# kerry-he/fsae-mpc

Measured on AMD Instinct MI355X. Metric: QP solves/sec (batched LTV-MPC, N=40 nx=5 nu=2 fp64), higher is better.
Workload: dtype f64

## Files before the change

fsae-mpc_amd/csrc/qp_solver.hip:

```cpp
#include <hip/hip_runtime.h>
#include <math.h>
#include <stdint.h>
#include <stdlib.h>
#include <stdio.h>
#include "qp_solver.h"

typedef double v4d __attribute__((ext_vector_type(4)));
typedef double v2d __attribute__((ext_vector_type(2)));

#define DEVINL __device__ __forceinline__
#ifndef QP_SOLVE_REFINE_STEPS
#define QP_SOLVE_REFINE_STEPS 1
#endif
#ifndef QP_FULL_BARRIERS
#define WAVE_SYNC() do { __builtin_amdgcn_fence(__ATOMIC_SEQ_CST, "wavefront"); __builtin_amdgcn_wave_barrier(); } while (0)
#else
#define WAVE_SYNC() __syncthreads()
#endif

namespace {

DEVINL double rl(double v, int src) {
  int lo = __builtin_amdgcn_readlane(__double2loint(v), src);
  int hi = __builtin_amdgcn_readlane(__double2hiint(v), src);
// ... 327 lines not shown
        int rank, size; group(k, on, rank, size);
        int base = on ? cnt[w][k] : 0;
        if (on) order[base + rank] = i0 + 64 * r + lane;
        if (on && rank == 0) cnt[w][k] = base + size;
      }
    }
}

#endif

struct Ctx {
  int n, m, T, Kq, J, JB, JT, np, ld, lane, c, q, nc, nb, ntr;
  const int* perm; const int* tcs; const int* aoff; const int* tend;
  const double* Aw; const double* Hw; const double* Ab; const double* Hb;
  double* rows;
  double* ring;
  double* cof;
  int rowlen;
  double* Ms;
  double* vec;
};
enum VecArr { V_X = 0, V_G, V_HX, V_R1, V_R2, V_P1, V_P2, V_P3, V_DX, V_E, V_NARR };

DEVINL double* rowp(const Ctx& k, int arr) { return k.rows + (size_t)arr * k.rowlen; }
DEVINL double* vecp(const Ctx& k, int arr) { return k.vec + arr * k.np; }

DEVINL bool row_valid(const Ctx& k, int js) {
  if (js < k.J) { const int s = 16 * js + k.c; return s < k.Kq && 4 * s + k.q < k.m; }
  return (js - k.J) * 64 + k.lane < k.n;
}

template <int T> DEVINL void hx_tiles(const Ctx& k, const double* X, double* HX) {
  double hx[T], hn[T][4], hc[T][4];
#pragma unroll
  for (int t = 0; t < T; ++t) hx[t] = 0.0;
#pragma unroll
  for (int Jt = 0; Jt < T; ++Jt)
#pragma unroll
    for (int p = 0; p < 4; ++p) hn[Jt][p] = k.Hw[((size_t)Jt * 4 + p) * 64 + k.lane];
#pragma unroll 1
  for (int I = 0; I < T; ++I) {
#pragma unroll
    for (int Jt = 0; Jt < T; ++Jt)
#pragma unroll
      for (int p = 0; p < 4; ++p) hc[Jt][p] = hn[Jt][p];
    if (I + 1 < T) {
#pragma unroll
      for (int Jt = 0; Jt < T; ++Jt)
#pragma unroll
        for (int p = 0; p < 4; ++p) hn[Jt][p] = k.Hw[((size_t)((I + 1) * T + Jt) * 4 + p) * 64 + k.lane];
    }
    double xk[4];
#pragma unroll
    for (int p = 0; p < 4; ++p) xk[p] = X[16 * I + k.q + 4 * p];
#pragma unroll
    for (int Jt = 0; Jt < T; ++Jt)
#pragma unroll
      for (int p = 0; p < 4; ++p) hx[Jt] = fma(hc[Jt][p], xk[p], hx[Jt]);
  }
#pragma unroll
  for (int t = 0; t < T; ++t) {
    double v = q_sum(hx[t]);
    if (k.q == 0) HX[16 * t + k.c] = v;
  }
}
template <int T> DEVINL void acc_init(const Ctx& k, v4d* acc) {
#pragma unroll
  for (int I = 0; I < T; ++I)
#pragma unroll
    for (int Jt = I; Jt < T; ++Jt) {
      const double* hp = k.Hw + ((size_t)(I * T + Jt) * 4) * 64 + k.lane;
      v4d h;
#pragma unroll
      for (int p = 0; p < 4; ++p) h[p] = hp[p * 64];
      acc[Tri<T>::idx(I, Jt)] = h;
    }
}

template <int T> DEVINL void hx_from_acc(const Ctx& k, const v4d* acc, const double* XV, double* HX) {
  double xr[T][4], xc[T], sc[T], sr[T][4];
#pragma unroll
  for (int I = 0; I < T; ++I) {
    xc[I] = XV[16 * I + k.c]; sc[I] = 0.0;
#pragma unroll
    for (int p = 0; p < 4; ++p) { xr[I][p] = XV[16 * I + k.q + 4 * p]; sr[I][p] = 0.0; }
  }
#pragma unroll
  for (int I = 0; I < T; ++I)
#pragma unroll
    for (int J = I; J < T; ++J) {
      const v4d& h = acc[Tri<T>::idx(I, J)];
#pragma unroll
      for (int p = 0; p < 4; ++p) {
        sc[J] = fma(h[p], xr[I][p], sc[J]);
        if (J > I) sr[I][p] = fma(h[p], xc[J], sr[I][p]);
      }
    }
  WAVE_SYNC();
#pragma unroll
  for (int J = 0; J < T; ++J) { const double v = q_sum(sc[J]); if (k.q == 0) HX[16 * J + k.c] = v; }
  WAVE_SYNC();
#pragma unroll
  for (int I = 0; I < T - 1; ++I)
#pragma unroll
    for (int p = 0; p < 4; ++p) { const double v = grp16_sum(sr[I][p]); if (k.c == 0) HX[16 * I + k.q + 4 * p] += v; }
}

template <int C> struct IC { static constexpr int value = C; };

#ifdef QP_DRAIN_STREAM
template <int T> struct StreamCfg {
  static constexpr int R = 3 * T;
};
template <int T> struct Stream {
  static constexpr int R = StreamCfg<T>::R;
  const char* gnext;
  int half;
  DEVINL void issue(const Ctx& k, int slot) {
    __builtin_amdgcn_global_load_lds((const __attribute__((address_space(1))) void*)(gnext + k.lane * 16),
                                     (__attribute__((address_space(3))) void*)(k.ring + slot * 128), 16, 0, 0);
    gnext += 1024;
  }
  DEVINL void start(const Ctx& k, int c0) {
    gnext = reinterpret_cast<const char*>(k.Aw); half = 0;
#pragma unroll
    for (int t = 0; t < T; ++t) if (t < c0) issue(k, t);
  }
  template <int C> DEVINL void next_pair(const Ctx& k, v2d* b, int cn) {
    asm volatile("s_waitcnt vmcnt(0)" ::: "memory");
    const int other = (half ^ 1) * T;
#pragma unroll
    for (int t = 0; t < T; ++t) if (t < cn) issue(k, other + t);
    asm volatile("" ::: "memory");
#pragma unroll
    for (int t = 0; t < C; ++t) b[t] = *reinterpret_cast<const v2d*>(k.ring + (half * T + t) * 128 + k.lane * 2);
    half ^= 1;
  }
  DEVINL void drain() { asm volatile("s_waitcnt vmcnt(0)" ::: "memory"); }
};
#else
template <int T> struct StreamCfg {
  static constexpr int D = 2 * T;
  static constexpr int R = D + T;
};
template <int T> struct Stream {
  static constexpr int D = StreamCfg<T>::D, R = StreamCfg<T>::R;
  const char* gnext; int slot_i, slot_e;
  DEVINL void issue(const Ctx& k) {
    __builtin_amdgcn_global_load_lds((const __attribute__((address_space(1))) void*)(gnext + k.lane * 16),
                                     (__attribute__((address_space(3))) void*)(k.ring + slot_i * 128), 16, 0, 0);
    gnext += 1024;
    slot_i = slot_i + 1 == R ? 0 : slot_i + 1;
  }
  DEVINL void start(const Ctx& k, int) {
    gnext = reinterpret_cast<const char*>(k.Aw); slot_i = 0; slot_e = 0;
#pragma unroll
    for (int j = 0; j < D; ++j) issue(k);
  }
  template <int C> DEVINL void next_pair(const Ctx& k, v2d* b, int) {
#pragma unroll
    for (int t = 0; t < C; ++t) issue(k);
    asm volatile("s_waitcnt vmcnt(%0)" :: "n"(D) : "memory");
#pragma unroll
    for (int t = 0; t < C; ++t) {
      int sl = slot_e + t; if (sl >= R) sl -= R;
      b[t] = *reinterpret_cast<const v2d*>(k.ring + sl * 128 + k.lane * 2);
    }
    slot_e += C; if (slot_e >= R) slot_e -= R;
  }
  DEVINL void drain() { asm volatile("s_waitcnt vmcnt(0)" ::: "memory"); }
};
#endif

template <int NA> struct CoefStage {
  double reg[NA > 0 ? NA : 1];
  DEVINL void load(const Ctx& k, const double* const* arr, int js) {
    const int jc = js < k.J ? js : k.J - 1;
#pragma unroll
    for (int a = 0; a < NA; ++a) reg[a] = arr[a][jc * 64 + k.lane];
  }
  DEVINL void commit(const Ctx& k) {
#pragma unroll
    for (int a = 0; a < NA; ++a) k.cof[a * 64 + k.lane] = reg[a];
  }
  DEVINL void read_pair(const Ctx& k, int s, v2d* out) const {
#pragma unroll
    for (int a = 0; a < NA; ++a) out[a] = *reinterpret_cast<const v2d*>(k.cof + a * 64 + k.q * 16 + (s & 15));
  }
};

template <int T, int NB> DEVINL void pass_syrk(const Ctx& k, v4d* acc, double* P1, double* P2, double* P3, double* MB) {
  constexpr int NBB = NB > 0 ? NB : 1;
  constexpr int NA = 4 + NB;
  const int JS = k.J * 64;
  const double* arr[NA];
  arr[0] = rowp(k, R_D); arr[1] = rowp(k, R_W1); arr[2] = rowp(k, R_W2); arr[3] = rowp(k, R_W3);
#pragma unroll
  for (int e = 0; e < NB; ++e) arr[4 + e] = k.Ab + (size_t)e * JS;
  double p1[T], p2[T], p3[T];
  double pb[NBB][T], sbb[NBB][NBB], pwb[3][NBB];
#pragma unroll
  for (int t = 0; t < T; ++t) { p1[t] = 0; p2[t] = 0; p3[t] = 0; }
#pragma unroll
  for (int e = 0; e < NBB; ++e) {
#pragma unroll
    for (int t = 0; t < T; ++t) pb[e][t] = 0;
#pragma unroll
    for (int f = 0; f < NBB; ++f) sbb[e][f] = 0;
    pwb[0][e] = pwb[1][e] = pwb[2][e] = 0;
  }
  Stream<T> st;
  CoefStage<NA> cs;
  int tr = 0;
  if (k.ntr > 0) { st.start(k, k.tcs[0]); cs.load(k, arr, 0); }
  auto phase = [&](auto Cc) __attribute__((always_inline)) {
    constexpr int C = decltype(Cc)::value;
    const int tr_end = k.tend[C];
    for (; tr < tr_end; ++tr) {
      if ((tr & 3) == 0) { cs.commit(k); cs.load(k, arr, (tr >> 2) + 1); }
#pragma unroll
      for (int u = 0; u < 2; ++u) {
        v2d b[C], cf[NA];
        st.template next_pair<C>(k, b, u == 0 ? C : (tr + 1 < tr_end ? C : (tr + 1 < k.ntr ? k.tcs[tr + 1] : 0)));
        cs.read_pair(k, 4 * tr + 2 * u, cf);
        asm volatile("" ::: "memory");
#pragma unroll
        for (int h = 0; h < 2; ++h) {
          double a[C], ab[NBB];
          const double dd = cf[0][h], w1 = cf[1][h], w2 = cf[2][h], w3 = cf[3][h];
#pragma unroll
          for (int e = 0; e < NB; ++e) ab[e] = cf[4 + e][h];
#pragma unroll
          for (int t = 0; t < C; ++t) a[t] = dd * b[t][h];
#pragma unroll
          for (int I = 0; I < C; ++I)
#pragma unroll
            for (int Jt = I; Jt < C; ++Jt)
              acc[Tri<T>::idx(I, Jt)] = __builtin_amdgcn_mfma_f64_16x16x4f64(a[I], b[Jt][h], acc[Tri<T>::idx(I, Jt)], 0, 0, 0);
#pragma unroll
          for (int t = 0; t < C; ++t) {
            p1[t] = fma(w1, b[t][h], p1[t]); p2[t] = fma(w2, b[t][h], p2[t]); p3[t] = fma(w3, b[t][h], p3[t]);
          }
#pragma unroll
          for (int e = 0; e < NB; ++e) {
            const double dab = dd * ab[e];
#pragma unroll
            for (int t = 0; t < C; ++t) pb[e][t] = fma(dab, b[t][h], pb[e][t]);
#pragma unroll
            for (int f = e; f < NB; ++f) sbb[e][f] = fma(dab, ab[f], sbb[e][f]);
            pwb[0][e] = fma(w1, ab[e], pwb[0][e]); pwb[1][e] = fma(w2, ab[e], pwb[1][e]); pwb[2][e] = fma(w3, ab[e], pwb[2][e]);
          }
        }
      }
    }
  };
  if constexpr (T >= 1) phase(IC<1>{});
  if constexpr (T >= 2) phase(IC<2>{});
  if constexpr (T >= 3) phase(IC<3>{});
  if constexpr (T >= 4) phase(IC<4>{});
  if constexpr (T >= 5) phase(IC<5>{});
  if constexpr (T >= 6) phase(IC<6>{});
  if constexpr (T >= 7) phase(IC<7>{});
  if constexpr (T >= 8) phase(IC<8>{});
  if (k.ntr > 0) st.drain();
#pragma unroll
  for (int t = 0; t < T; ++t) {
    double v1 = q_sum(p1[t]), v2 = q_sum(p2[t]), v3 = q_sum(p3[t]);
    if (k.q == 0) { P1[16 * t + k.c] = v1; P2[16 * t + k.c] = v2; P3[16 * t + k.c] = v3; }
  }
#pragma unroll
  for (int e = 0; e < NB; ++e) {
#pragma unroll
    for (int t = 0; t < T; ++t) { const double vb = q_sum(pb[e][t]); if (k.q == 0) MB[e * k.np + 16 * t + k.c] = vb; }
    const double v1 = q_sum(pwb[0][e]), v2 = q_sum(pwb[1][e]), v3 = q_sum(pwb[2][e]);
    if (k.lane == 0) { P1[k.nc + e] = v1; P2[k.nc + e] = v2; P3[k.nc + e] = v3; }
#pragma unroll
    for (int f = 0; f < NB; ++f) {
      const double sv = q_sum(f >= e ? sbb[e][f] : sbb[f][e]);
      if (k.lane == 0) MB[e * k.np + k.nc + f] = sv;
    }
  }
}

template <int T, int NB, int NVEC, int FUSE> DEVINL void pass_Av(const Ctx& k, const double* const* vin, double* const* rout, double* Pcor, double* Pcor2 = nullptr, const double* const* cfarr = nullptr) {
  constexpr int NBB = NB > 0 ? NB : 1;
  constexpr int NC = FUSE == 1 ? 6 : (FUSE >= 2 ? 3 : 0);
  constexpr int NA = NC + NB;
  const int JS = k.J * 64;
  const double* arr[NA > 0 ? NA : 1];
  if (FUSE == 1) { arr[0] = rowp(k, R_RPL); arr[1] = rowp(k, R_CB1); arr[2] = rowp(k, R_CC1); arr[3] = rowp(k, R_RPU); arr[4] = rowp(k, R_CB2); arr[5] = rowp(k, R_CC2); }
  if (FUSE >= 2) { arr[0] = cfarr ? cfarr[0] : rowp(k, R_CB1); arr[1] = cfarr ? cfarr[1] : rowp(k, R_RPL); arr[2] = cfarr ? cfarr[2] : rowp(k, R_CC1); }
#pragma unroll
  for (int f = 0; f < NB; ++f) arr[NC + f] = k.Ab + (size_t)f * JS;
  double v[NVEC][T], vb[NVEC][NBB], pc[T], pcb[NBB], pd[FUSE >= 2 ? T : 1], pdb[NBB];
#pragma unroll
  for (int e = 0; e < NVEC; ++e) {
#pragma unroll
    for (int t = 0; t < T; ++t) v[e][t] = vin[e][16 * t + k.c];
#pragma unroll
    for (int f = 0; f < NB; ++f) vb[e][f] = vin[e][k.nc + f];
  }
#pragma unroll
  for (int t = 0; t < T; ++t) pc[t] = 0.0;
#pragma unroll
  for (int f = 0; f < NBB; ++f) { pcb[f] = 0.0; pdb[f] = 0.0; }
#pragma unroll
  for (int t = 0; t < (FUSE >= 2 ? T : 1); ++t) pd[t] = 0.0;
  double keep[NVEC + 1];
#pragma unroll
  for (int e = 0; e < NVEC + 1; ++e) keep[e] = 0.0;
  Stream<T> st;
  CoefStage<NA> cs;
  int tr = 0;
  if (k.ntr > 0) { st.start(k, k.tcs[0]); if (NA > 0) cs.load(k, arr, 0); }
  auto phase = [&](auto Cc) __attribute__((always_inline)) {
    constexpr int C = decltype(Cc)::value;
    const int tr_end = k.tend[C];
    for (; tr < tr_end; ++tr) {
      if (NA > 0 && (tr & 3) == 0) { cs.commit(k); cs.load(k, arr, (tr >> 2) + 1); }
#pragma unroll
      for (int u = 0; u < 2; ++u) {
        v2d b[C], cf[NA > 0 ? NA : 1];
        st.template next_pair<C>(k, b, u == 0 ? C : (tr + 1 < tr_end ? C : (tr + 1 < k.ntr ? k.tcs[tr + 1] : 0)));
// ... 364 lines not shown
  k.aoff = k.tcs + d.ntr; k.tend = k.aoff + d.ntr + 1;
  extern __shared__ double lds[];
  k.Ms = nullptr; k.vec = lds;
  double* MB = lds + (size_t)V_NARR * d.np;
  double* YL = MB + (size_t)(NB > 0 ? NB : 1) * d.np;
  k.ring = YL + T * 272;
  k.cof = k.ring + StreamCfg<T>::R * 128;
  double* SCR = k.ring;
  const double* gw = ws + d.off_gw;
  const double* Es = ws + d.off_E;
  const double* Fs = ws + d.off_F;
  const int lane = k.lane, n = k.n, JT = k.JT, J = k.J, nc = k.nc, nb = k.nb;
  constexpr int NT = Tri<T>::NT;
  constexpr int NBB = NB > 0 ? NB : 1;

#define X vecp(k, V_X)
#define G vecp(k, V_G)
#define HX vecp(k, V_HX)
#define R1 vecp(k, V_R1)
#define R2 vecp(k, V_R2)
#define P1 vecp(k, V_P1)
#define P2 vecp(k, V_P2)
#define P3 vecp(k, V_P3)
#define DX vecp(k, V_DX)
#define EV vecp(k, V_E)
#define aL rowp(k, R_L)
#define aU rowp(k, R_U)
#define aTL rowp(k, R_TL)
#define aTU rowp(k, R_TU)
#define aZL rowp(k, R_ZL)
#define aZU rowp(k, R_ZU)
#define aV rowp(k, R_V)
#define aD rowp(k, R_D)
#define aW1 rowp(k, R_W1)
#define aW2 rowp(k, R_W2)
#define aW3 rowp(k, R_W3)
#define aVA rowp(k, R_VA)
#define aVC rowp(k, R_VC)
#define aRPL rowp(k, R_RPL)
#define aRPU rowp(k, R_RPU)

  auto hx_border = [&](const double* XV) __attribute__((always_inline)) {
    if (NB > 0) {
      WAVE_SYNC();
      double xb[NBB], sb[NBB];
#pragma unroll
      for (int e = 0; e < NB; ++e) { xb[e] = XV[nc + e]; sb[e] = 0.0; }
      for (int h = 0; h < 2; ++h) {
        const int i = lane + 64 * h;
        if (i < n) {
          double add = 0.0;
#pragma unroll
          for (int e = 0; e < NB; ++e) { const double hbi = k.Hb[(size_t)e * k.np + i]; add = fma(hbi, xb[e], add); sb[e] = fma(hbi, XV[i], sb[e]); }
          if (i < nc) HX[i] += add;
        }
      }
#pragma unroll
      for (int e = 0; e < NB; ++e) { const double tot = wave_sum(sb[e]); if (lane == 0) HX[nc + e] = tot; }
    }
  };
  auto hx_full = [&](const double* XV) __attribute__((always_inline)) { hx_tiles<T>(k, XV, HX); hx_border(XV); };

  for (int i = lane; i < k.np; i += 64) { G[i] = gw[i]; EV[i] = Es[i]; R1[i] = 0; R2[i] = 0; DX[i] = 0; }
  int cnt_local = 0, infeas = 0;
  for (int js = 0; js < JT; ++js) {
    const int ix = js * 64 + lane;
    const bool valid = row_valid(k, js);
    double l = aL[ix], u = aU[ix];
    if (valid) {
      if (l > -INFINITY && u < INFINITY) {
        if (l > u) infeas = 1;
        if (!(u > l)) {
          const double eps = 1e-9 * fmax(1.0, fabs(l));
          l -= eps; u += eps; aL[ix] = l; aU[ix] = u;
        }
      }
      cnt_local += (l > -INFINITY) + (u < INFINITY);
    }
    if (js >= J) {
      const int i = (js - J) * 64 + lane;
      if (i < k.np) {
        double xi = 0.0;
        if (P.x_init) { const int ui = i < k.n ? qp_user_index(d, i) : -1; if (ui >= 0) { const double xs = P.x_init[(size_t)b * d.nu + ui] / EV[i]; if (fabs(xs) < INFINITY) xi = xs; } }
        if (valid) { if (l > -INFINITY && xi < l) xi = l; if (u < INFINITY && xi > u) xi = u; }
        X[i] = xi;
      }
    }
  }
  const double cnt = fmax(1.0, wave_sum((double)cnt_local));
  infeas = wave_max((double)infeas) > 0;
  WAVE_SYNC();

  STAMP_DECL
  int flag = 1, it = 0, flag_polished = 0;
  double fval_s = 0.0, merit_s = INFINITY;
  if (infeas) { flag = -2; }
  if (ws[d.off_bad] != 0.0) flag = -1;

  {
    const double* vin[1] = {X}; double* rout[1] = {aV};
    pass_Av<T, NB, 1, 0>(k, vin, rout, nullptr);
    for (int jb = 0; jb < k.JB; ++jb) { const int i = jb * 64 + lane; aV[(J + jb) * 64 + lane] = i < n ? X[i] : 0.0; }
  }
  const double T0 = 10.0, Z0 = 100.0;
  for (int js = 0; js < JT; ++js) {
    const int ix = js * 64 + lane;
    const bool valid = row_valid(k, js);
    const double l = aL[ix], u = aU[ix], v = aV[ix];
    const bool hl = valid && l > -INFINITY, hu = valid && u < INFINITY;
    aTL[ix] = hl ? fmax(v - l, T0) : 1.0;
    aTU[ix] = hu ? fmax(u - v, T0) : 1.0;
    aZL[ix] = hl ? Z0 : 0.0;
    aZU[ix] = hu ? Z0 : 0.0;
    aW3[ix] = (js < J) ? ((hl ? Z0 : 0.0) - (hu ? Z0 : 0.0)) : 0.0;
  }
  WAVE_SYNC();
  {
    hx_full(X);
    pass_Atw<T, NB>(k, aW3, P3);
    WAVE_SYNC();
    for (int jb = 0; jb < k.JB; ++jb) {
      const int i = jb * 64 + lane, ix = (J + jb) * 64 + lane;
      if (i < n) {
        const double r = HX[i] + G[i] - P3[i];
        if (aL[ix] > -INFINITY) aZL[ix] = fmax(r, 0.0) + Z0;
        if (aU[ix] < INFINITY) aZU[ix] = fmax(-r, 0.0) + Z0;
      }
    }
    WAVE_SYNC();
  }

  double saved_merit = INFINITY, best_res = INFINITY;
  int have_saved = 0, stall = 0;
  double* XS = ws + d.off_save;
  double* LAMS = ws + d.off_save + k.np;

  auto row1_body = [&](int ix, bool valid, double l, double u, double v, double tl, double tu, double zl, double zu,
                       double& s_gap, double& m_rp) {
    const bool hl = valid && l > -INFINITY, hu = valid && u < INFINITY;
    const double rpl = hl ? v - l - tl : 0.0, rpu = hu ? u - v - tu : 0.0;
    const double dl_ = hl ? zl / tl : 0.0, du_ = hu ? zu / tu : 0.0;
    aRPL[ix] = rpl; aRPU[ix] = rpu;
    rowp(k, R_CB1)[ix] = dl_; rowp(k, R_CC1)[ix] = hl ? dl_ / tl : 0.0;
    rowp(k, R_CB2)[ix] = du_; rowp(k, R_CC2)[ix] = hu ? du_ / tu : 0.0;
    aD[ix] = dl_ + du_;
    aW1[ix] = -dl_ * rpl + du_ * rpu;
    aW2[ix] = (hl ? 1.0 / tl : 0.0) - (hu ? 1.0 / tu : 0.0);
    aW3[ix] = (hl ? zl : 0.0) - (hu ? zu : 0.0);
    s_gap += (hl ? tl * zl : 0.0) + (hu ? tu * zu : 0.0);
    const double sc = fmax(1.0, fabs(v));
    if (hl) m_rp = fmax(m_rp, fabs(rpl) / fmax(sc, fabs(l)));
    if (hu) m_rp = fmax(m_rp, fabs(rpu) / fmax(sc, fabs(u)));
  };
  struct Slot { int ix; bool valid; double l, u, v, tl, tu, zl, zu, va, vc, w2, rpl, rpu; };
  auto load_slot = [&](int js) {
    Slot s_;
    const int jc = js < JT ? js : JT - 1;
    s_.ix = jc * 64 + lane; s_.valid = js < JT && row_valid(k, jc);
    const int ix = s_.ix;
    s_.l = aL[ix]; s_.u = aU[ix]; s_.v = aV[ix]; s_.tl = aTL[ix]; s_.tu = aTU[ix]; s_.zl = aZL[ix]; s_.zu = aZU[ix];
    s_.va = aVA[ix]; s_.vc = aVC[ix]; s_.w2 = aW2[ix]; s_.rpl = aRPL[ix]; s_.rpu = aRPU[ix];
    return s_;
  };
  double gap = 0.0, rp_rel = 0.0;

  v4d acc[NT];
  v4d rh[T];
  double Ubb[NBB][NBB];
  auto border_solve = [&](double* R) __attribute__((always_inline)) {
    if (NB > 0) {
      double yb[NBB], xb[NBB];
#pragma unroll
      for (int e = 0; e < NB; ++e) {
        double dsum = 0.0;
        for (int h = 0; h < 2; ++h) { const int i = lane + 64 * h; if (i < nc) dsum = fma(MB[e * k.np + i], R[i], dsum); }
        double tt = R[nc + e] - wave_sum(dsum);
#pragma unroll
        for (int g2 = 0; g2 < e; ++g2) tt -= Ubb[g2][e] * yb[g2];
        yb[e] = tt / Ubb[e][e];
      }
#pragma unroll
      for (int e = NB - 1; e >= 0; --e) {
        double tt = yb[e];
#pragma unroll
        for (int f = e + 1; f < NB; ++f) tt -= Ubb[e][f] * xb[f];
        xb[e] = tt / Ubb[e][e];
      }
      WAVE_SYNC();
      for (int h = 0; h < 2; ++h) {
        const int i = lane + 64 * h;
        if (i < nc) {
          double r = R[i];
#pragma unroll
          for (int e = 0; e < NB; ++e) r = fma(-MB[e * k.np + i], xb[e], r);
          R[i] = r;
        }
      }
      if (lane == 0) {
#pragma unroll
        for (int e = 0; e < NB; ++e) R[nc + e] = xb[e];
      }
      WAVE_SYNC();
    }
  };
  auto factor_solve2 = [&](int it_now) __attribute__((always_inline)) -> int {
    double dmax_l = 0;
#pragma unroll
    for (int K = 0; K < T; ++K) {
      const int i = 16 * K + k.c;
      const int ix = (J + (i >> 6)) * 64 + (i & 63);
      const double dadd = i < n ? aD[ix] : 1.0;
      const bool mine = (k.q == (k.c & 3));
#pragma unroll
      for (int p = 0; p < 4; ++p)
        if (mine && p == (k.c >> 2)) { acc[Tri<T>::idx(K, K)][p] += dadd; dmax_l = fmax(dmax_l, acc[Tri<T>::idx(K, K)][p]); }
    }
    if (NB > 0) {
      for (int h = 0; h < 2; ++h) {
        const int i = lane + 64 * h;
        if (i < k.np) {
          const int ix = (J + (i >> 6)) * 64 + (i & 63);
#pragma unroll
          for (int e = 0; e < NB; ++e) {
            double v = i < n ? k.Hb[(size_t)e * k.np + i] + MB[e * k.np + i] : 0.0;
            if (i == nc + e) { v += e < nb ? aD[ix] : 1.0; dmax_l = fmax(dmax_l, v); }
            MB[e * k.np + i] = v;
          }
        }
      }
    }
    const double dmax = wave_max(dmax_l);
    WAVE_SYNC();
#ifdef QP_DEBUG_DUMP
    if (P.dump && b == 0 && P.dump_stage == 1 && it_now == P.dump_iter) {
#pragma unroll
      for (int I = 0; I < T; ++I)
#pragma unroll
        for (int Jt = I; Jt < T; ++Jt)
#pragma unroll
          for (int p = 0; p < 4; ++p) {
            const int r = 16 * I + k.q + 4 * p, cc = 16 * Jt + k.c;
            if (r < n && cc < n) { P.dump[r * n + cc] = acc[Tri<T>::idx(I, Jt)][p]; if (I != Jt || cc >= r) P.dump[cc * n + r] = acc[Tri<T>::idx(I, Jt)][p]; }
          }
      for (int e = 0; e < nb; ++e)
        for (int i = lane; i < n; i += 64) { P.dump[i * n + nc + e] = MB[e * k.np + i]; P.dump[(nc + e) * n + i] = MB[e * k.np + i]; }
      for (int i = lane; i < n; i += 64) { P.dump[n * n + i] = P1[i]; P.dump[n * n + n + i] = P2[i]; P.dump[n * n + 2 * n + i] = P3[i]; P.dump[n * n + 3 * n + i] = HX[i]; }
    }
#endif
#ifdef QP_MFMA_SOLVES
    {
      const double* vin[6] = {R1, R2, MB, MB + k.np, MB + 2 * k.np, MB + 3 * k.np};
      rhs_load<T, 2 + NB>(k, rh, vin);
    }
    int fbad = reg_factor<T>(k, acc, YL, rh, 1e-30 * dmax);
#else
    int fbad = reg_factor_only<T>(k, acc, YL, 1e-30 * dmax);
    WAVE_SYNC();
    STAMP(5);
#endif
    if (NB > 0) {
#ifdef QP_MFMA_SOLVES
      double* vout[6] = {R1, R2, MB, MB + k.np, MB + 2 * k.np, MB + 3 * k.np};
      rhs_store<T, 2 + NB>(k, rh, vout);
      WAVE_SYNC();
#else
#pragma unroll
      for (int e = 0; e < NB; ++e) {
        double ue[T][4];
        vec_forward<T, true>(k, acc, YL, MB + e * k.np, ue);
        WAVE_SYNC();
        vec_rows_store<T>(k, ue, MB + e * k.np);
      }
      WAVE_SYNC();
#endif
      double S[NBB][NBB];
#pragma unroll
      for (int e = 0; e < NB; ++e)
#pragma unroll
        for (int f = e; f < NB; ++f) {
          double dsum = 0.0;
          for (int h = 0; h < 2; ++h) { const int i = lane + 64 * h; if (i < nc) dsum = fma(MB[e * k.np + i], MB[f * k.np + i], dsum); }
          S[e][f] = MB[e * k.np + nc + f] - wave_sum(dsum);
        }
#pragma unroll
      for (int e = 0; e < NB; ++e) {
        double dd = S[e][e];
#pragma unroll
        for (int g2 = 0; g2 < e; ++g2) dd -= Ubb[g2][e] * Ubb[g2][e];
        if (!(dd > 1e-30 * dmax)) { if (!(fabs(dd) < INFINITY)) fbad = 1; dd = 1e-30 * dmax; }
        Ubb[e][e] = sqrt(dd);
#pragma unroll
        for (int f = e + 1; f < NB; ++f) {
          double tt = S[e][f];
#pragma unroll
          for (int g2 = 0; g2 < e; ++g2) tt -= Ubb[g2][e] * Ubb[g2][f];
          Ubb[e][f] = tt / Ubb[e][e];
        }
      }
    }
    if (fbad) return 1;
#ifdef QP_MFMA_SOLVES
    if (NB > 0) {
      border_solve(R1); border_solve(R2);
      const double* vin[2] = {R1, R2};
      rhs_load<T, 2>(k, rh, vin);
    }
// ... 85 lines not shown
        const double sc = fmax(1.0, fmax(fabs(G[i]), fmax(fabs(HX[i]), fabs(gz))));
        m_rd = fmax(m_rd, fabs(HX[i] + G[i] - gz) / sc);
      }
    }
    const double fval = wave_sum(fl);
    const double rd_rel = wave_max(m_rd);
    const double gap_rel = gap / fmax(1.0, fabs(fval));
    const double merit = (fabs(fval) < INFINITY && fabs(gap_rel) < INFINITY) ? fmax(rd_rel, fmax(rp_rel, gap_rel)) : INFINITY;
    fval_s = fval; merit_s = merit;
    const bool res_ok = merit <= P.tol;
#ifdef QP_DEBUG_DUMP
    if (P.dump && P.dump_stage == 5 && b == P.dump_iter && lane == 0 && it < 120) {
      double* o_ = P.dump + 16 * it;
      o_[0] = merit; o_[1] = rd_rel; o_[2] = rp_rel; o_[3] = gap_rel; o_[4] = mu; o_[5] = fval; o_[6] = (double)have_saved; o_[7] = saved_merit;
    }
#endif
    if (!(merit < INFINITY)) { flag = have_saved ? 2 : -1; break; }
    if (merit <= P.tol_loose && merit < saved_merit) {
      for (int i = lane; i < k.np; i += 64) XS[i] = X[i];
      for (int js = 0; js < JT; ++js) LAMS[js * 64 + lane] = aW3[js * 64 + lane];
      have_saved = 1; saved_merit = merit;
    } else if (merit > P.tol_loose && rp_rel <= P.tol_loose && gap_rel <= P.tol_loose) {
      double dgap = 0, m_rd2 = 0, lamfix[2] = {0.0, 0.0};
      for (int h = 0; h < 2; ++h) {
        const int i = lane + 64 * h;
        if (i < n) {
          const int ix = (J + (i >> 6)) * 64 + (i & 63);
          const double lam = aW3[ix], gz = P3[i] + lam, r = HX[i] + G[i] - gz;
          const double lam2 = lam + r, l = aL[ix], u = aU[ix], v = aV[ix];
          const bool ok = lam2 >= 0 ? l > -INFINITY : u < INFINITY;
          if (ok) { lamfix[h] = lam2; dgap += fabs(r) * fmax(0.0, lam2 >= 0 ? v - l : u - v); }
          else {
            lamfix[h] = lam;
            const double sc = fmax(1.0, fmax(fabs(G[i]), fmax(fabs(HX[i]), fabs(gz))));
            m_rd2 = fmax(m_rd2, fabs(r) / sc);
          }
        }
      }
      const double merit2 = fmax(wave_max(m_rd2), fmax(rp_rel, (gap + wave_sum(dgap)) / fmax(1.0, fabs(fval))));
      if (merit2 <= P.tol_loose && merit2 < saved_merit) {
        for (int i = lane; i < k.np; i += 64) XS[i] = X[i];
        for (int js = 0; js < J; ++js) LAMS[js * 64 + lane] = aW3[js * 64 + lane];
        for (int h = 0; h < 2; ++h) { const int i = lane + 64 * h; if (i < k.np) LAMS[(J + (i >> 6)) * 64 + (i & 63)] = i < n ? lamfix[h] : 0.0; }
        have_saved = 1; saved_merit = merit2;
      }
      if (have_saved) { flag = 2; break; }
    } else if (have_saved && merit > P.tol_loose) { flag = 2; break; }
    if (merit < 0.9 * best_res) { best_res = merit; stall = 0; } else ++stall;

    for (int h = 0; h < 2; ++h) {
      const int i = lane + 64 * h;
      if (i < k.np) {
        const int ix = (J + (i >> 6)) * 64 + (i & 63);
        R1[i] = i < n ? -(HX[i] + G[i]) + P1[i] + aW1[ix] : 0.0;
        R2[i] = i < n ? P2[i] + aW2[ix] : 0.0;
      }
    }
    STAMP(4);
    if (factor_solve2(it)) {
      flag = (res_ok || have_saved) ? 2 : -1;
      if (flag == -1 && P.polish && rp_rel <= QP_BREAKDOWN_TRY_TOL && gap_rel <= QP_BREAKDOWN_TRY_TOL) flag = 4;
      break;
    }
    STAMP(6);
#ifdef QP_DEBUG_DUMP
    if (P.dump && b == 0 && P.dump_stage == 2 && it == P.dump_iter) {
      for (int i = lane; i < n; i += 64) { P.dump[i] = R1[i]; P.dump[n + i] = R2[i]; }
    }
#endif
    if (res_ok) {
      double dm = 0, xm = 1.0;
      for (int h = 0; h < 2; ++h) {
        const int i = lane + 64 * h;
        if (i < n) { dm = fmax(dm, fabs(R1[i] * EV[i])); xm = fmax(xm, fabs(X[i] * EV[i])); }
      }
      dm = wave_max(dm); xm = wave_max(xm);
      if (dm <= P.tol_x * xm) { flag = 0; break; }
    }
    if (it >= P.max_iter) { flag = have_saved ? 2 : 1; break; }

    {
      const double* vin[2] = {R1, R2}; double* rout[2] = {aVA, aVC};
      pass_Av<T, NB, 2, 1>(k, vin, rout, P1);
      for (int jb = 0; jb < k.JB; ++jb) {
        const int i = jb * 64 + lane;
        aVA[(J + jb) * 64 + lane] = i < n ? R1[i] : 0.0;
        aVC[(J + jb) * 64 + lane] = i < n ? R2[i] : 0.0;
      }
    }
    STAMP(7);
    double a_aff = 1.0, s1 = 0.0, s2 = 0.0;
    auto row2_body = [&](const Slot& r, int js) {
      const bool hl = r.valid && r.l > -INFINITY, hu = r.valid && r.u < INFINITY;
      double w = 0.0;
      if (hl) {
        const double dt = r.va + r.rpl, dz = -r.zl - (r.zl / r.tl) * dt;
        if (dt < 0) a_aff = fmin(a_aff, -r.tl / dt);
        if (dz < 0) a_aff = fmin(a_aff, -r.zl / dz);
        s1 += r.tl * dz + r.zl * dt; s2 += dt * dz;
        w -= dt * dz / r.tl;
      }
      if (hu) {
        const double dt = -r.va + r.rpu, dz = -r.zu - (r.zu / r.tu) * dt;
        if (dt < 0) a_aff = fmin(a_aff, -r.tu / dt);
        if (dz < 0) a_aff = fmin(a_aff, -r.zu / dz);
        s1 += r.tu * dz + r.zu * dt; s2 += dt * dz;
        w += dt * dz / r.tu;
      }
      if (js >= J && js < JT) aW1[r.ix] = w;
    };
    for (int js = 0; js < JT; js += 2) {
      const Slot r0 = load_slot(js), r1 = load_slot(js + 1);
      row2_body(r0, js); row2_body(r1, js + 1);
    }
    a_aff = wave_min(a_aff);
    s1 = wave_sum(s1); s2 = wave_sum(s2);
    const double mu_aff = fmax(0.0, gap + a_aff * (s1 + a_aff * s2)) / cnt;
    double sigma = mu > 0 ? (mu_aff / mu) * (mu_aff / mu) * (mu_aff / mu) : 0.0;
    if (sigma > 1.0) sigma = 1.0;
    {
      const double mu_floor = 1e-5 * P.tol * fmax(1.0, fabs(fval)) / cnt;
      if (mu > 0 && sigma < mu_floor / mu) sigma = fmin(1.0, mu_floor / mu);
    }
    const double smu = sigma * mu;
    const double cw = a_aff >= 0.05 ? 1.0 : 0.0;
    WAVE_SYNC();
    STAMP(8);
    if (cw != 0.0) {
    STAMP(9);
    for (int h = 0; h < 2; ++h) {
      const int i = lane + 64 * h;
      if (i < k.np) { const int ix = (J + (i >> 6)) * 64 + (i & 63); DX[i] = i < n ? P1[i] + aW1[ix] : 0.0; }
    }
    WAVE_SYNC();
    solve1(DX);
    WAVE_SYNC();
    STAMP(10);
    {
      const double* vin[1] = {DX}; double* rout[1] = {aW2};
      pass_Av<T, NB, 1, 0>(k, vin, rout, nullptr);
      for (int jb = 0; jb < k.JB; ++jb) { const int i = jb * 64 + lane; aW2[(J + jb) * 64 + lane] = i < n ? DX[i] : 0.0; }
    }
    STAMP(11);
    } else {
      for (int i = lane; i < k.np; i += 64) DX[i] = 0.0;
      for (int js = 0; js < JT; ++js) aW2[js * 64 + lane] = 0.0;
      WAVE_SYNC();
    }
    for (int h = 0; h < 2; ++h) {
      const int i = lane + 64 * h;
      if (i < n) DX[i] = R1[i] + smu * R2[i] + DX[i];
    }
    double amax = 1e300, bp = 0, bdp = 0, bd = 0, bdd = 0, q1 = 0.0, q2 = 0.0;
    auto row3a_body = [&](const Slot& r, int js) {
      const bool hl = r.valid && r.l > -INFINITY, hu = r.valid && r.u < INFINITY;
      const double dv = r.va + smu * r.vc + r.w2;
      if (js < JT) aVC[r.ix] = dv;
      if (hl) {
        const double dta = r.va + r.rpl, dza = -r.zl - (r.zl / r.tl) * dta;
        const double cl = smu - cw * dta * dza;
        const double dt = dv + r.rpl, dz = -r.zl + cl / r.tl - (r.zl / r.tl) * dt;
        if (dt < 0 && -r.tl / dt < amax) { amax = -r.tl / dt; bp = r.tl; bdp = dt; bd = r.zl; bdd = dz; }
        if (dz < 0 && -r.zl / dz < amax) { amax = -r.zl / dz; bp = r.zl; bdp = dz; bd = r.tl; bdd = dt; }
        q1 += r.tl * dz + r.zl * dt; q2 += dt * dz;
      }
      if (hu) {
        const double dta = -r.va + r.rpu, dza = -r.zu - (r.zu / r.tu) * dta;
        const double cu = smu - cw * dta * dza;
        const double dt = -dv + r.rpu, dz = -r.zu + cu / r.tu - (r.zu / r.tu) * dt;
        if (dt < 0 && -r.tu / dt < amax) { amax = -r.tu / dt; bp = r.tu; bdp = dt; bd = r.zu; bdd = dz; }
        if (dz < 0 && -r.zu / dz < amax) { amax = -r.zu / dz; bp = r.zu; bdp = dz; bd = r.tu; bdd = dt; }
        q1 += r.tu * dz + r.zu * dt; q2 += dt * dz;
      }
    };
    for (int js = 0; js < JT; js += 2) {
      const Slot r0 = load_slot(js), r1 = load_slot(js + 1);
      row3a_body(r0, js); row3a_body(r1, js + 1);
    }
    const double amax_w = wave_min(amax);
    double alpha = 1.0;
    if (amax_w < 1e299) {
      const unsigned long long msk = __ballot(amax == amax_w);
      const int src = __ffsll((long long)msk) - 1;
      bp = rl(bp, src); bdp = rl(bdp, src); bd = rl(bd, src); bdd = rl(bdd, src);
      q1 = wave_sum(q1); q2 = wave_sum(q2);
      const double gamma_f = 0.99, gamma_a = 1.0 / (1.0 - gamma_f);
      const double mufull = fmax(0.0, gap + amax_w * (q1 + amax_w * q2)) / cnt / gamma_a;
      const double a_h = (-bp + mufull / (bd + amax_w * bdd)) / bdp;
      alpha = fmin(1.0, fmin(0.99999999 * amax_w, fmax(a_h, gamma_f * amax_w)));
    }
#ifdef QP_DEBUG_DUMP
    if (P.dump && P.dump_stage == 5 && b == P.dump_iter && lane == 0 && it < 120) {
      double* o_ = P.dump + 16 * it;
      o_[8] = a_aff; o_[9] = sigma; o_[10] = alpha; o_[11] = cw; o_[12] = amax_w; o_[13] = (double)stall;
    }
    if (P.dump && b == 0 && P.dump_stage == 4 && it == P.dump_iter) {
      double c1 = 0, c2 = 0, c3 = 0, c4 = 0;
      for (int js = 0; js < JT; ++js) { const int ix = js * 64 + lane; c1 += aVA[ix]; c2 += aVC[ix]; c3 += aW2[ix]; c4 += aW1[ix]; }
      c1 = wave_sum(c1); c2 = wave_sum(c2); c3 = wave_sum(c3); c4 = wave_sum(c4);
      if (lane == 0) {
        double* o_ = P.dump;
        o_[0] = a_aff; o_[1] = mu_aff; o_[2] = sigma; o_[3] = smu; o_[4] = cw; o_[5] = amax_w; o_[6] = alpha; o_[7] = gap; o_[8] = mu;
        o_[9] = c1; o_[10] = c2; o_[11] = c3; o_[12] = c4; o_[13] = s1; o_[14] = s2; o_[15] = q1; o_[16] = q2;
      }
      for (int i = lane; i < n; i += 64) { P.dump[32 + i] = DX[i]; P.dump[32 + n + i] = R1[i]; P.dump[32 + 2 * n + i] = R2[i]; P.dump[32 + 3 * n + i] = P1[i]; }
    }
#endif
    double xn = 0, zn = 0, s_gap = 0, m_rp = 0;
    auto row3b_body = [&](const Slot& r, int js) {
      if (js >= JT) return;
      const bool hl = r.valid && r.l > -INFINITY, hu = r.valid && r.u < INFINITY;
      const double dv = r.vc;
      double tl = r.tl, zl = r.zl, tu = r.tu, zu = r.zu;
      if (hl) {
        const double dta = r.va + r.rpl, dza = -zl - (zl / tl) * dta;
        const double cl = smu - cw * dta * dza;
        const double dt = dv + r.rpl, dz = -zl + cl / tl - (zl / tl) * dt;
        tl += alpha * dt; zl += alpha * dz;
        aTL[r.ix] = tl; aZL[r.ix] = zl;
        zn = fmax(zn, zl);
      }
      if (hu) {
        const double dta = -r.va + r.rpu, dza = -zu - (zu / tu) * dta;
        const double cu = smu - cw * dta * dza;
        const double dt = -dv + r.rpu, dz = -zu + cu / tu - (zu / tu) * dt;
        tu += alpha * dt; zu += alpha * dz;
        aTU[r.ix] = tu; aZU[r.ix] = zu;
        zn = fmax(zn, zu);
      }
      const double v = r.v + alpha * dv;
      aV[r.ix] = v;
      row1_body(r.ix, r.valid, r.l, r.u, v, tl, tu, zl, zu, s_gap, m_rp);
    };
    for (int js = 0; js < JT; js += 2) {
      const Slot r0 = load_slot(js), r1 = load_slot(js + 1);
      row3b_body(r0, js); row3b_body(r1, js + 1);
    }
    for (int h = 0; h < 2; ++h) {
      const int i = lane + 64 * h;
      if (i < n) { X[i] += alpha * DX[i]; xn = fmax(xn, fabs(X[i])); }
    }
    const double rp_prev = rp_rel;
    gap = wave_sum(s_gap);
    rp_rel = wave_max(m_rp);
    xn = wave_max(xn); zn = wave_max(zn);
    WAVE_SYNC();
    STAMP(12);
    if (xn > 1e13) { flag = rp_prev > 1e-6 ? -2 : (fval < -1e13 ? -3 : -1); break; }
    if (zn > 1e15 && rp_prev > 1e-6) { flag = -2; break; }
    if (stall > (have_saved ? 5 : 25)) { flag = have_saved ? 2 : (rp_prev > 1e-6 ? -2 : (P.polish ? 5 : 1)); break; }
  }

  const bool v_current = flag == 0 || flag == 4;
  if (flag == 2) {
    for (int i = lane; i < k.np; i += 64) X[i] = XS[i];
    for (int js = 0; js < JT; ++js) aW3[js * 64 + lane] = LAMS[js * 64 + lane];
    flag = 0; merit_s = saved_merit;
    WAVE_SYNC();
  } else {
    for (int js = 0; js < JT; ++js) {
      const int ix = js * 64 + lane;
      const bool valid = row_valid(k, js);
      const bool hl = valid && aL[ix] > -INFINITY, hu = valid && aU[ix] < INFINITY;
      aW3[ix] = (hl ? aZL[ix] : 0.0) - (hu ? aZU[ix] : 0.0);
    }
    WAVE_SYNC();
  }
#ifdef QP_DEBUG_DUMP
  if (P.dump && P.dump_stage == 5 && b == P.dump_iter && lane == 0) { double* o_ = P.dump + 16 * 120; o_[4] = (double)flag; for (int i_ = 5; i_ < 48; ++i_) o_[i_] = 0.0; }
#endif
  if ((flag == 0 || flag == 4 || flag == 5) && P.polish) {
    const double rho = 1e6, pin = 1e16, rinv = 1.0 / rho;
    double* PA = rowp(k, R_CB1); double* PB = rowp(k, R_RPL); double* PY = rowp(k, R_CC1); double* PS = rowp(k, R_CB2);
    double* PC = rowp(k, R_RPU); double* PP = rowp(k, R_CC2); double* PZ0 = aW2;
    double* ATR = R1; double* ATP = P3;
    if (!v_current) {
      const double* vin[1] = {X}; double* rout[1] = {aV};
      pass_Av<T, NB, 1, 0>(k, vin, rout, nullptr);
      for (int jb = 0; jb < k.JB; ++jb) { const int i = jb * 64 + lane; aV[(J + jb) * 64 + lane] = i < n ? X[i] : 0.0; }
    }
    for (int js = 0; js < JT; ++js) {
      const int ix = js * 64 + lane;
      const bool valid = row_valid(k, js);
      const double l = aL[ix], u = aU[ix], v = aV[ix], lam = aW3[ix];
      const bool lo = valid && l > -INFINITY && lam > 0 && lam > fabs(v - l);
      const bool up = valid && u < INFINITY && lam < 0 && -lam > fabs(u - v);
      PS[ix] = lo ? 1.0 : (up ? -1.0 : 0.0); PY[ix] = ((lo || up) && js < J) ? lam : 0.0;
    }
    for (int i = lane; i < k.np; i += 64) XS[i] = X[i];
    WAVE_SYNC();
    for (int attempt = 0; attempt < QP_REFINE_ATTEMPTS && flag_polished <= 0; ++attempt) {
    for (int js = 0; js < JT; ++js) {
      const int ix = js * 64 + lane;
      const double sd = PS[ix];
      PA[ix] = sd != 0.0 ? rho : 0.0; PB[ix] = sd > 0 ? aL[ix] : (sd < 0 ? aU[ix] : 0.0);
      aD[ix] = js < J ? PA[ix] : (sd != 0.0 ? pin : 0.0); aW1[ix] = 0.0; aW2[ix] = 0.0; PC[ix] = 0.0; PP[ix] = 0.0;
    }
    WAVE_SYNC();
    acc_init<T>(k, acc);
    pass_syrk<T, NB>(k, acc, P1, P2, P3, MB);
    WAVE_SYNC();
    for (int i = lane; i < k.np; i += 64) { R1[i] = 0.0; R2[i] = 0.0; }
    WAVE_SYNC();
    bool pok = factor_solve2(-1) == 0, retry = false;
    if (!pok) { flag_polished = -5; break; }
    for (int h = 0; h < 2; ++h) {
      const int i = lane + 64 * h;
      if (i < k.np) { const int ix = (J + (i >> 6)) * 64 + (i & 63); R2[i] = (i < n && PS[ix] != 0.0) ? PB[ix] : XS[i]; }
    }
    WAVE_SYNC();
    const double* cf_eval[3] = {PA, PB, PY};
    const double* cf_cg[3] = {PA, PZ0, PZ0};
    auto eval_zy = [&]() __attribute__((always_inline)) {
      const double* vin[1] = {R2}; double* rout[2] = {aVA, aVC};
      pass_Av<T, NB, 1, 3>(k, vin, rout, P1, P2, cf_eval);
      hx_full(R2);
      WAVE_SYNC();
    };
    if (pok) {
      eval_zy();
      for (int h = 0; h < 2; ++h) {
        const int i = lane + 64 * h;
        if (i < k.np) { const int ix = (J + (i >> 6)) * 64 + (i & 63); DX[i] = (i < n && PS[ix] == 0.0) ? -(HX[i] + G[i] - P1[i]) : 0.0; }
      }
      WAVE_SYNC();
      solve1(DX);
      WAVE_SYNC();
      for (int h = 0; h < 2; ++h) {
        const int i = lane + 64 * h;
        if (i < n) { const int ix = (J + (i >> 6)) * 64 + (i & 63); if (PS[ix] == 0.0) R2[i] += DX[i]; }
      }
      WAVE_SYNC();
      eval_zy();
      double rs_l = 0.0;
      for (int js = 0; js < J; ++js) {
        const int ix = js * 64 + lane;
        const double cc_ = PA[ix] != 0.0 ? aVA[ix] - PB[ix] : 0.0;
        PC[ix] = cc_; PP[ix] = -cc_; rs_l = fma(cc_, cc_, rs_l);
      }
      double rs = wave_sum(rs_l);
      for (int h = 0; h < 2; ++h) { const int i = lane + 64 * h; if (i < k.np) { ATR[i] = -P2[i] * rinv; ATP[i] = ATR[i]; } }
      WAVE_SYNC();
      for (int cgit = 0; cgit < 12 && pok; ++cgit) {
        double m_eq = 0.0, m_cy = 0.0;
        for (int js = 0; js < J; ++js) {
          const int ix = js * 64 + lane;
          m_eq = fmax(m_eq, fabs(PC[ix]) / fmax(1.0, fabs(PB[ix])));
          m_cy = fmax(m_cy, fabs(PC[ix] * PY[ix]));
        }
        m_eq = wave_max(m_eq); m_cy = wave_max(m_cy);
        if (m_eq <= 1e-11 && m_cy <= 1e-11 * fmax(1.0, fabs(fval_s))) break;
        if (cgit == 11) { pok = false; flag_polished = -6; break; }
        for (int h = 0; h < 2; ++h) {
          const int i = lane + 64 * h;
          if (i < k.np) { const int ix = (J + (i >> 6)) * 64 + (i & 63); DX[i] = (i < n && PS[ix] == 0.0) ? ATP[i] : 0.0; }
        }
        WAVE_SYNC();
        solve1(DX);
        WAVE_SYNC();
        {
          const double* vin[1] = {DX}; double* rout[2] = {aVA, aVC};
          pass_Av<T, NB, 1, 3>(k, vin, rout, P1, P2, cf_cg);
        }
        WAVE_SYNC();
        double pq_l = 0.0;
        for (int js = 0; js < J; ++js) { const int ix = js * 64 + lane; if (PA[ix] != 0.0) pq_l = fma(PP[ix], aVA[ix], pq_l); }
        const double pq = wave_sum(pq_l);
        if (!(pq > 0.0) || !(rs > 0.0)) {
          pok = false; flag_polished = -7;
          if (attempt < QP_REFINE_ATTEMPTS - 1) {
            double my = 0.0; int myix = -1;
            for (int js = 0; js < J; ++js) { const int ix = js * 64 + lane; if (PA[ix] != 0.0 && fabs(PP[ix]) > my) { my = fabs(PP[ix]); myix = ix; } }
            const double mx = wave_max(my);
            if (mx > 0.0 && my == mx && myix >= 0) { PS[myix] = 0.0; PY[myix] = 0.0; }
            for (int i = lane; i < k.np; i += 64) XS[i] = R2[i];
            WAVE_SYNC();
            retry = true;
          }
          break;
        }
        const double alpha_ = rs / pq;
        double rsn_l = 0.0;
        for (int js = 0; js < J; ++js) {
          const int ix = js * 64 + lane;
          if (PA[ix] != 0.0) {
            PY[ix] = fma(alpha_, PP[ix], PY[ix]);
            const double cc_ = fma(alpha_, aVA[ix], PC[ix]);
// ... 504 lines not shown
```

Measured before the change: 374,800.

## Bound stream prefetch to matrix extent and keep leading row slots in registers

The LDS streaming prefetcher now counts the remaining matrix chunks and stops issuing global-to-LDS loads past the end of the data. It picks the matching vmcnt wait from the number of loads actually outstanding, and drain becomes a no-op. Separately, for small T the first two row slots loaded in the step-length pass are kept in registers, along with their computed dv, and reused in the update pass instead of being reloaded from memory. This cuts wasted overrun loads and some repeated slot loads, at the cost of more branching in the stream code and higher register pressure.

```diff
diff --git a/fsae-mpc_amd/csrc/qp_solver.hip b/fsae-mpc_amd/csrc/qp_solver.hip
--- a/fsae-mpc_amd/csrc/qp_solver.hip
+++ b/fsae-mpc_amd/csrc/qp_solver.hip
@@ -503,15 +503,46 @@
     gnext += 1024;
     slot_i = slot_i + 1 == R ? 0 : slot_i + 1;
   }
+#ifdef QP_STREAM_OVERRUN
   DEVINL void start(const Ctx& k, int) {
     gnext = reinterpret_cast<const char*>(k.Aw); slot_i = 0; slot_e = 0;
 #pragma unroll
     for (int j = 0; j < D; ++j) issue(k);
   }
-  template <int C> DEVINL void next_pair(const Ctx& k, v2d* b, int) {
+  template <int C> DEVINL void request(const Ctx& k) {
 #pragma unroll
     for (int t = 0; t < C; ++t) issue(k);
     asm volatile("s_waitcnt vmcnt(%0)" :: "n"(D) : "memory");
+  }
+  DEVINL void drain() { asm volatile("s_waitcnt vmcnt(0)" ::: "memory"); }
+#else
+  int rem, skipped;
+  DEVINL void issue_or_skip(const Ctx& k) { if (rem > 0) { issue(k); --rem; } else ++skipped; }
+  template <int N> static DEVINL void wait_outstanding(int n) {
+    if constexpr (N == 0) asm volatile("s_waitcnt vmcnt(0)" ::: "memory");
+    else { if (n >= N) asm volatile("s_waitcnt vmcnt(%0)" :: "n"(N) : "memory"); else wait_outstanding<N - 1>(n); }
+  }
+  DEVINL void start(const Ctx& k, int) {
+    gnext = reinterpret_cast<const char*>(k.Aw); slot_i = 0; slot_e = 0;
+    rem = k.aoff[k.ntr]; skipped = 0;
+#pragma unroll
+    for (int j = 0; j < D; ++j) issue_or_skip(k);
+  }
+  template <int C> DEVINL void request(const Ctx& k) {
+    if (rem >= C) {
+#pragma unroll
+      for (int t = 0; t < C; ++t) issue(k);
+      rem -= C;
+    } else {
+#pragma unroll
+      for (int t = 0; t < C; ++t) issue_or_skip(k);
+    }
+    wait_outstanding<D>(D - skipped);
+  }
+  DEVINL void drain() { }
+#endif
+  template <int C> DEVINL void next_pair(const Ctx& k, v2d* b, int) {
+    request<C>(k);
 #pragma unroll
     for (int t = 0; t < C; ++t) {
       int sl = slot_e + t; if (sl >= R) sl -= R;
@@ -519,7 +550,6 @@
     }
     slot_e += C; if (slot_e >= R) slot_e -= R;
   }
-  DEVINL void drain() { asm volatile("s_waitcnt vmcnt(0)" ::: "memory"); }
 };
 #endif
 
@@ -1190,6 +1220,12 @@
     if (hl) m_rp = fmax(m_rp, fabs(rpl) / fmax(sc, fabs(l)));
     if (hu) m_rp = fmax(m_rp, fabs(rpu) / fmax(sc, fabs(u)));
   };
+#ifdef QP_ROW3_KEEP
+  constexpr int ROW3_KEEP = QP_ROW3_KEEP;
+#else
+  constexpr int ROW3_KEEP = T <= 5 ? 2 : 0;
+#endif
+  static_assert(ROW3_KEEP >= 0 && ROW3_KEEP % 2 == 0, "QP_ROW3_KEEP: even");
   struct Slot { int ix; bool valid; double l, u, v, tl, tu, zl, zu, va, vc, w2, rpl, rpu; };
   auto load_slot = [&](int js) {
     Slot s_;
@@ -1581,7 +1617,7 @@
       if (i < n) DX[i] = R1[i] + smu * R2[i] + DX[i];
     }
     double amax = 1e300, bp = 0, bdp = 0, bd = 0, bdd = 0, q1 = 0.0, q2 = 0.0;
-    auto row3a_body = [&](const Slot& r, int js) {
+    auto row3a_body = [&](const Slot& r, int js) -> double {
       const bool hl = r.valid && r.l > -INFINITY, hu = r.valid && r.u < INFINITY;
       const double dv = r.va + smu * r.vc + r.w2;
       if (js < JT) aVC[r.ix] = dv;
@@ -1601,8 +1637,14 @@
         if (dz < 0 && -r.zu / dz < amax) { amax = -r.zu / dz; bp = r.zu; bdp = dz; bd = r.tu; bdd = dt; }
         q1 += r.tu * dz + r.zu * dt; q2 += dt * dz;
       }
+      return dv;
     };
-    for (int js = 0; js < JT; js += 2) {
+    Slot kept[ROW3_KEEP > 0 ? ROW3_KEEP : 1];
+#pragma unroll
+    for (int c = 0; c < ROW3_KEEP; ++c) if (c < JT) kept[c] = load_slot(c);
+#pragma unroll
+    for (int c = 0; c < ROW3_KEEP; ++c) if (c < JT) kept[c].vc = row3a_body(kept[c], c);
+    for (int js = ROW3_KEEP; js < JT; js += 2) {
       const Slot r0 = load_slot(js), r1 = load_slot(js + 1);
       row3a_body(r0, js); row3a_body(r1, js + 1);
     }
@@ -1661,7 +1703,9 @@
       aV[r.ix] = v;
       row1_body(r.ix, r.valid, r.l, r.u, v, tl, tu, zl, zu, s_gap, m_rp);
     };
-    for (int js = 0; js < JT; js += 2) {
+#pragma unroll
+    for (int c = 0; c < ROW3_KEEP; ++c) if (c < JT) row3b_body(kept[c], c);
+    for (int js = ROW3_KEEP; js < JT; js += 2) {
       const Slot r0 = load_slot(js), r1 = load_slot(js + 1);
       row3b_body(r0, js); row3b_body(r1, js + 1);
     }
```

After: 353,600, median of 2. 0.944x the previous value.
